# mlodel/gym-exploration-2d

Hardware: AMD Instinct MI355X
Metric: env-steps/sec (whole node), 4096 worlds x 10 agents (higher is better)
Workload: dtype f64; 1 GPU; 4096 worlds x 10 agents per GPU, RVO/ORCA on-device LP policy + OtherAgentsStates sensor, UnicycleDynamics, random-goal episodes with auto-reset (BASELINE configs[2]); worlds_per_gpu=4096, agents=10, launch_mode=cagym_rollout, parallelism=worlds sharded x1, no data-path collective

## Files before the change

### gym-exploration-2d_amd/csrc/cagym_api.hip

```cpp
#include <hip/hip_runtime.h>
#include <cmath>
#include <cstdio>
#include <cstdlib>
#include <algorithm>
#include <cstring>
#include <string>
#include <vector>

#include "../../include/cagym.h"
#include "cagym_gen1.h"
#include "cagym_sensors.h"
#include "cagym_kernels3.h"
#include "cagym_split3.h"
#include "cagym_launch3.h"
#ifdef CAGYM_MONOLITHIC
#include "cagym_k3_all.inc"
#endif
#include "cagym_ig.h"
#include "cagym_ga3c.h"
#include "cagym_ga3c16.h"
#include "cagym_gen.h"
#include "cagym_gen2.h"
#include "cagym_dmcts.h"
#include "cagym_ig_episode.h"
// ... 10 lines not shown
struct Env {
    cagym_config cfg;
    CagymDev D;
    std::vector<void*> allocs;
    std::string err;
    bool scenarios_set = false;
    double* sc_obst = nullptr;
    float4* sc_obst_prep = nullptr;
    double* sc_heading_buf = nullptr;
    IgDev G{};
    uint32_t* ig_any = nullptr;
    IgEpisode ig_ep{};
    int32_t* gen_failed = nullptr;
    int32_t* ga3c_ctr = nullptr;
    unsigned char* ga3c_packed = nullptr;
    const float* ga3c_packed_src = nullptr;
    int32_t* status_host = nullptr;
    bool ig_ready = false;
    int any_rvo = 1;
    int obst_rvo = 0;
    int generation = 3;
    int wpw10 = 5;
    size_t pre_lds_min = 0;
    bool begun = false;
    EpRec rec{};
    bool rec_ready = false;
    EpLog elog{};
    bool log_ready = false;
    void* elog_ring = nullptr;
    int n_ig = 0;
    bool streaming = false;
    StreamDev stream{};
    cagym_gen2_params stream_P{};
};
enum { N_IG_UNEQUAL = -1, N_IG_RANDOM = -2 };

int fail(Env* e, int code, const std::string& msg) {
    g_last_error = msg;
    if (e) e->err = msg;
    return code;
}

#define HIPCHK(e, call)                                                                              \
    do {                                                                                             \
        hipError_t _s = (call);                                                                      \
        if (_s != hipSuccess)                                                                        \
            return fail(e, CAGYM_E_HIP, std::string(#call) + ": " + hipGetErrorString(_s));          \
    } while (0)

struct DeviceGuard {
    int prev = -1;
    bool switched = false;
    hipError_t status = hipSuccess;
    explicit DeviceGuard(int dev) {
        status = hipGetDevice(&prev);
        if (status == hipSuccess && prev != dev) {
            status = hipSetDevice(dev);
            switched = status == hipSuccess;
        }
    }
    ~DeviceGuard() {
        if (switched) (void)hipSetDevice(prev);
    }
};
#define ENTRY_IF(e, env, state_ok, msg)                                \
    Env* e = reinterpret_cast<Env*>(env);                              \
    if (!e) return fail(nullptr, CAGYM_E_INVALID, "null env");         \
    if (!(state_ok)) return fail(e, CAGYM_E_STATE, msg)
#define ENTRY(e, env) ENTRY_IF(e, env, true, "")
#define ENTRY_POOL(e, env, name) ENTRY_IF(e, env, e->scenarios_set, name " before cagym_set_scenarios")
#define ENTRY_IG(e, env, name) ENTRY_IF(e, env, e->ig_ready, name " before cagym_ig_init")
#define ON_DEVICE(e)                                                                                       \
    DeviceGuard _guard((e)->cfg.device);                                                                   \
    if (_guard.status != hipSuccess) return fail(e, CAGYM_E_HIP, std::string("hipSetDevice: ") + hipGetErrorString(_guard.status)); \
    if (int _rc = device_status(e)) return _rc
#define ON_DEVICE_VOIDS_BEGUN(e) \
    ON_DEVICE(e);                \
    (e)->begun = false

int device_status(Env* e) {
    const int32_t code = e->status_host ? *reinterpret_cast<volatile int32_t*>(e->status_host) : 0;
    if (code == CAGYM_DEVERR_NONE) return CAGYM_OK;
    return fail(e, CAGYM_E_DEVICE, std::string("a kernel of an earlier launch gave up a bounded wait (") +
                                       (code == CAGYM_DEVERR_LP_WAIT ? "LP waves" : code == CAGYM_DEVERR_LASER_WAIT ? "LaserScan passes" : "unknown") +
                                       "): results since then are void, destroy the handle");
}

template <typename T>
int dalloc(Env* e, T** p, size_t n) {
    void* q = nullptr;
    size_t bytes = (n ? n : 1) * sizeof(T);
    hipError_t s = hipMalloc(&q, bytes);
    if (s != hipSuccess) return fail(e, CAGYM_E_NOMEM, std::string("hipMalloc: ") + hipGetErrorString(s));
    s = hipMemset(q, 0, bytes);
    if (s != hipSuccess) return fail(e, CAGYM_E_HIP, std::string("hipMemset: ") + hipGetErrorString(s));
    e->allocs.push_back(q);
    *p = reinterpret_cast<T*>(q);
    return CAGYM_OK;
}

CagymOut to_out(const Env* e, const cagym_outputs* o, bool scan_as_given = false) {
    CagymOut r{};
    if (o) {
        r.obs_oas = o->obs_oas;
        r.obs_ego = o->obs_ego;
        r.laserscan = (e->cfg.laserscan || scan_as_given) ? o->laserscan : nullptr;
        r.reward = o->reward;
        r.flags = o->flags;
        r.game_over = o->game_over;
    }
    return r;
}

#define WPW20 2
#define NT20 256
struct Spec2 {
    int nt, mt, wpw;
};
inline Spec2 spec2(int M, int wpw10) {
    if (M == 10) return {256, 10, wpw10};
    if (M == 4) return {256, 4, 0};
    if (M == 20) return {NT20, 20, WPW20};
    if (M <= 12) return {256, 0, 0};
    return {512, 0, 0};
}
inline Spec2 spec2(const Env* e) { return spec2(e->cfg.max_agents, e->wpw10); }
inline int wpw_spec(const Env* e) { return spec2(e).wpw; }
inline int n_wg2(const Env* e) {
    const int M = e->cfg.max_agents;
    const int wpw = wpw_spec(e) ? wpw_spec(e) : CAGYM_WAVE / M;
    return (e->cfg.n_worlds + wpw - 1) / wpw;
}
inline size_t lds3_bytes(const cagym_config& cfg, const Spec2 sp, bool obst, bool lines) {
    const int M = cfg.max_agents;
    return cagym_lds3_bytes(M, cagym_as(M, sp.wpw), sp.nt, (obst && lines) ? 2 * cfg.max_obstacles : 0, cagym_lpl3(sp.mt, obst), obst, sp.mt);
}
inline size_t lds3_bytes(const Env* e, bool obst, bool lines) { return lds3_bytes(e->cfg, spec2(e), obst, lines); }
inline bool has_map(const Env* e) { return e->cfg.max_obstacles > 0; }
inline size_t scan_bytes(const Env* e) { return (size_t)e->cfg.n_worlds * e->cfg.max_agents * 16 * sizeof(float); }
inline size_t lds3_bytes(const Env* e) { return lds3_bytes(e, has_map(e), e->obst_rvo != 0); }
inline size_t lds3_step_bytes(const Env* e) {
    if (!has_map(e)) return lds3_bytes(e);
    return cagym_lds3_ovl_bytes(e->cfg.max_agents, cagym_as(e->cfg.max_agents, wpw_spec(e)), spec2(e).nt, e->D.ko);
}
inline int lp_group_width(const Env* e) {
    const int mt = spec2(e).mt;
    return cagym_gw3(mt);
}

inline int n_waves(const Env* e) {
    int wpw = CAGYM_WAVE / e->cfg.max_agents;
    return (e->cfg.n_worlds + wpw - 1) / wpw;
}

struct K3Entry {
    int nt, mt, wp;
    void (*launch[2])(const K3Launch&);
    void (*setattr[2])(int);
};
#define K3_ROW(NT, MT, WP)                                                                     \
    {NT, MT, WP, {cagym_k3_launch_##NT##_##MT##_##WP##_0, cagym_k3_launch_##NT##_##MT##_##WP##_1}, \
     {cagym_k3_setattr_##NT##_##MT##_##WP##_0, cagym_k3_setattr_##NT##_##MT##_##WP##_1}},
const K3Entry k3_table[] = {CAGYM_K3_SPECS(K3_ROW)};
#undef K3_ROW
inline const K3Entry* k3_entry(const Env* e) {
    const Spec2 sp = spec2(e);
    for (const K3Entry& r : k3_table)
// ... 1444 lines not shown
```

### gym-exploration-2d_amd/csrc/cagym_kernels3.h

```cpp
#pragma once
#include "cagym_device.h"
#include "cagym_orca.h"

#include "cagym_spin.h"
#include "cagym_trace.h"

#ifndef CAGYM_GW10
#define CAGYM_GW10 8
#endif

__host__ __device__ inline size_t a16(size_t x) { return (x + 15) & ~(size_t)15; }

__device__ __forceinline__ void prio_chain3(bool lagging) {
#ifndef CAGYM_NO_LAG_PRIORITY
    if (lagging) __builtin_amdgcn_s_setprio(3);
    else __builtin_amdgcn_s_setprio(1);
#endif
}
__device__ __forceinline__ void prio_rows3() {
#ifndef CAGYM_NO_LAG_PRIORITY
    __builtin_amdgcn_s_setprio(0);
#endif
}
__host__ __device__ constexpr int cagym_gw3(int MT) { return MT > 0 && MT <= 5 ? 4 : (MT > 0 && MT <= 10 ? CAGYM_GW10 : 16); }
// ... 498 lines not shown
        if (!skip) gp = d - cr;
        klo = d - rl - rh;
        khi = d - rh - rl;
        const float rpx = (float)phx - (float)plx, rpy = (float)phy - (float)ply;
        dq = rpx * rpx + rpy * rpy;
    }
    W.hit[lo * MP + shi] = ht;
    W.hit[hi * MP + slo] = ht;
    if (GAP && gp < INFINITY) atomicMin(&W.gmin[lo], gap_key(gp));
    W.keys[lo * MP + shi] = klo;
    W.keys[hi * MP + slo] = khi;
    if (DSQ) {
        W.dsq[lo * MP + shi] = make_uint2((uint32_t)shi, __float_as_uint(dq));
        W.dsq[hi * MP + slo] = make_uint2((uint32_t)slo, __float_as_uint(dq));
    }
}

template <int MT>
__device__ __forceinline__ void pair_dsq3(const Lds3& W, int p, int M, int MP) {
    const UPair q = upair_of<MT>(p, M);
    const int n = W.wn[q.wl];
    const int lo = q.wl * M + (q.i < q.j ? q.i : q.j), hi = q.wl * M + (q.i < q.j ? q.j : q.i);
    const int slo = lo - q.wl * M, shi = hi - q.wl * M;
    float dq = INFINITY;
    if (shi < n) {
        const float rpx = (float)W.tpx[hi] - (float)W.tpx[lo], rpy = (float)W.tpy[hi] - (float)W.tpy[lo];
        dq = rpx * rpx + rpy * rpy;
    }
    W.dsq[lo * MP + shi] = make_uint2((uint32_t)shi, __float_as_uint(dq));
    W.dsq[hi * MP + slo] = make_uint2((uint32_t)slo, __float_as_uint(dq));
}

template <int MT>
__device__ __forceinline__ int neighbour_rank3(const Lds3& W, int a, int sl, float dq, int MP) {
    const uint4* row = reinterpret_cast<const uint4*>(W.dsq + a * MP);
    const unsigned long long me = ((unsigned long long)__float_as_uint(dq) << 32) | (unsigned)sl;
    int rank = 0;
    constexpr int MPT = MT > 0 ? ((MT + 1) & ~1) : 0;
    if (MT > 0) {
#pragma unroll
        for (int l2 = 0; l2 < MPT; l2 += 2) {
            const uint4 v = row[l2 >> 1];
            rank += ((((unsigned long long)v.y << 32) | v.x) < me) ? 1 : 0;
            rank += ((((unsigned long long)v.w << 32) | v.z) < me) ? 1 : 0;
        }
    } else {
        for (int l2 = 0; l2 < MP; l2 += 2) {
            const uint4 v = row[l2 >> 1];
            rank += ((((unsigned long long)v.y << 32) | v.x) < me) ? 1 : 0;
            rank += ((((unsigned long long)v.w << 32) | v.z) < me) ? 1 : 0;
        }
    }
    return rank;
}

template <int MT>
__device__ __forceinline__ void half_planes3(const CagymDev& D, const Lds3& W, int p, int M, int MP, int AS, int ko) {
    const UPair q = upair_of<MT>(p, M);
    const int n = W.wn[q.wl];
    const int a = q.wl * M + q.i, b = q.wl * M + q.j;
    const bool both = q.i < n && q.j < n;
    const bool on_a = both && W.trvo[a] != 0;
    const bool on_b = both && W.trvo[b] != 0;
    if (!(on_a || on_b)) return;
    const float vax = (float)W.tvx[a], vay = (float)W.tvy[a];
    const OrcaPair g = orca_pair((float)W.tpx[a], (float)W.tpy[a], vax, vay, (float)((1 + 15e-2) * W.tr[a]), (float)D.dt,
                                 W.tpx[b], W.tpy[b], W.tvx[b], W.tvy[b], W.tr[b]);
    PMARK("hp_pair_done");
    if (on_a) {
        const float c = W.tcoop[a];
        const float4 ln = make_float4(vax + c * g.ux, vay + c * g.uy, g.zx, g.zy);
        const float2 s0 = W.lpc[a];
        if (detf(ln.z, ln.w, ln.x - s0.x, ln.y - s0.y) > 0.0f) W.busy[a] = 1;
        const int rank = neighbour_rank3<MT>(W, a, q.j, g.d2, MP);
        if (rank < D.maxnb) W.sorted[(ko + rank) * AS + a] = ln;
    }
    if (on_b) {
        const float c = W.tcoop[b];
        const float4 ln = make_float4((float)W.tvx[b] - c * g.ux, (float)W.tvy[b] - c * g.uy, -g.zx, -g.zy);
        const float2 s0 = W.lpc[b];
        if (detf(ln.z, ln.w, ln.x - s0.x, ln.y - s0.y) > 0.0f) W.busy[b] = 1;
        const int rank = neighbour_rank3<MT>(W, b, q.i, g.d2, MP);
        if (rank < D.maxnb) W.sorted[(ko + rank) * AS + b] = ln;
    }
}

__device__ __forceinline__ void oas_row3(const Lds3& W, float* oas_out, int p, int npairs, int M, int MP, int K, int wpw,
                                         int worlds_valid, uint32_t inv_m) {
    PMARK("oas_begin");
    if (p >= npairs) return;
    const PairIdx q = pair_of(p, M, inv_m);
    if (q.j == q.sl || q.wl >= worlds_valid) return;
    const int n = W.wn[q.wl];
    float* my = oas_out + ((size_t)blockIdx.x * wpw * M + q.a) * K * 10;
    const double kj = W.keys[q.a * MP + q.j];
    if (!(kj > -INFINITY)) {
        const int row = q.sl < n ? q.j - 1 : (q.j < q.sl ? q.j : q.j - 1);
        float2* r2 = reinterpret_cast<float2*>(my + row * 10);
        const float2 z = make_float2(0.f, 0.f);
#pragma unroll
        for (int c = 0; c < 5; c++) r2[c] = z;
        return;
    }
    int before = 0;
    const double2* krow = reinterpret_cast<const double2*>(W.keys + q.a * MP);
    for (int l2 = 0; l2 < M; l2 += 2) {
        const double2 kk = krow[l2 >> 1];
        before += (kk.x > kj) || (kk.x == kj && l2 + 0 > q.j);
        before += (kk.y > kj) || (kk.y == kj && l2 + 1 > q.j);
    }
    const int row = before;
    PMARK("oas_ranked");
    const int b = q.a - q.sl + q.j;
    const double dx = W.tpx[b] - W.tpx[q.a], dy = W.tpy[b] - W.tpy[q.a];
    const double prx = W.tprx[q.a], pry = W.tpry[q.a], orx = -pry, ory = prx;
    const double ovx = W.tvx[b], ovy = W.tvy[b], orad = W.tr[b];
    float v[10];
    v[0] = (float)dx;
    v[1] = (float)dy;
    v[2] = (float)dot2(dx, dy, prx, pry);
    v[3] = (float)dot2(dx, dy, orx, ory);
    v[4] = (float)dot2(ovx, ovy, prx, pry);
    v[5] = (float)dot2(ovx, ovy, orx, ory);
    v[6] = (float)orad;
    v[7] = (float)(W.tr[q.a] + orad);
    v[8] = (float)kj;
    v[9] = ST_POLICY(W.tst[b]) == CAGYM_POL_STATIC ? 1.f : 2.f;
    PMARK("oas_store");
    float2* r2 = reinterpret_cast<float2*>(my + row * 10);
#pragma unroll
    for (int c = 0; c < 5; c++) r2[c] = make_float2(v[2 * c], v[2 * c + 1]);
}

__device__ __forceinline__ void ego_obs3(const CagymDev& D, const Lds3& W, float* ego_out, int a, int M, int wpw, uint32_t inv_m) {
    if (a >= wpw * M) return;
    const int wl = (int)__umulhi((uint32_t)a, inv_m);
    const int slot = a - wl * M;
    const int world = blockIdx.x * wpw + wl;
    if (world >= D.N) return;
    const int n = W.wn[wl];
    const bool active = slot < n;
    const int nobs = active ? n - 1 : 0;
    const size_t aidx = (size_t)world * M + slot;
    D.n_observed[aidx] = nobs;
    if (!ego_out) return;
    float4* e = reinterpret_cast<float4*>(ego_out + aidx * CAGYM_EGO_WIDTH);
    if (active) {
        const double px = W.tpx[a], py = W.tpy[a];
        e[0] = make_float4((float)W.tdg[a], (float)(W.tgx[a] - px), (float)(W.tgy[a] - py), (float)W.tr[a]);
        e[1] = make_float4((float)W.the[a], (float)W.th[a], (float)px, (float)py);
        e[2] = make_float4((float)W.tpref[a], (float)nobs, ST_POLICY(W.tst[a]) == CAGYM_POL_LEARNING ? 1.f : 0.f, 0.f);
    } else {
        const float4 z = make_float4(0.f, 0.f, 0.f, 0.f);
        e[0] = z; e[1] = z; e[2] = z;
    }
}

template <bool LEAN>
__device__ __forceinline__ bool sample_cell(double x, double y, int& gx, int& gy) {
    if (!LEAN) return world_to_cell(x, y, gx, gy);
    const double qy = y * 10.0, qx = x * 10.0;
    const bool safe = fabs(qy - rint(qy)) > 1e-7 && fabs(qx - rint(qx)) > 1e-7 && fabs(qy) < 1e6 && fabs(qx) < 1e6;
    if (!safe) return world_to_cell(x, y, gx, gy);
    gx = (int)floor((30 / 2.) / 0.1 - qy);
    gy = (int)floor((30 / 2.) / 0.1 + qx);
    return gx >= 0 && gy >= 0 && gx < CAGYM_MAPD && gy < CAGYM_MAPD;
// ... 118 lines not shown
            rng[i] = (uint8_t)((klo << 4) | khi);
        }
        cnt[c] = (uint8_t)__popcll(m);
    }
    WGTRACE_W1(30);
    if (!lds_wait_ge(&W.flag[8], npass)) *D.dev_status = CAGYM_DEVERR_LASER_WAIT;
    int n = 0;
    for (int q = 0; q < npass; q++) n += cnt[q];
    WGTRACE_W1_VALUE(32, n);
    for (;;) {
        int r = 0;
        if (lane == 0) r = __hip_atomic_fetch_add(&W.flag[10], 1, __ATOMIC_RELAXED, __HIP_MEMORY_SCOPE_WORKGROUP);
        r = __builtin_amdgcn_readlane(r, 0);
        if (r * CAGYM_WAVE >= n) break;
        int i = r * CAGYM_WAVE + lane;
        if (i < n) {
            int q = 0;
            for (; q < npass; q++) {
                const int cq = cnt[q];
                if (i < cq) break;
                i -= cq;
            }
            const int e = lst[q * CAGYM_WAVE + i], kk = rng[q * CAGYM_WAVE + i];
            const int a = e >> 4, b = e & 15;
            const int wl = (int)__umulhi((uint32_t)a, inv_m);
            const int slot = a - wl * M;
            const int world = blockIdx.x * wpw + wl;
            const uint32_t* map = D.map_bits + (size_t)W.wsc[wl] * CAGYM_MAPD * CAGYM_MAPW;
            laser_out[((size_t)world * M + slot) * 16 + b] = laserscan_beam_range<BATCH>(map, W.tpx[a], W.tpy[a], W.th[a], W.tr[a], b, kk >> 4, kk & 15);
        }
    }
    WGTRACE_W1(31);
}

template <bool OBST, int BATCH = 8>
__device__ __forceinline__ void observation_chunks3(const CagymDev& D, const Lds3& W, const CagymOut& o, int npairs, int M, int MP,
                                                    int K, int wpw, int worlds_valid, uint32_t inv_m, int ko = 0, int AS = 0) {
    const int lane = threadIdx.x & (CAGYM_WAVE - 1);
    const int nck = (npairs + CAGYM_WAVE - 1) / CAGYM_WAVE;
    for (;;) {
        int c = 0;
        if (lane == 0) c = __hip_atomic_fetch_add(&W.flag[1], 1, __ATOMIC_RELAXED, __HIP_MEMORY_SCOPE_WORKGROUP);
        c = __builtin_amdgcn_readlane(c, 0);
        if (c > nck) break;
        if (c < nck) {
            if (o.obs_oas) oas_row3(W, o.obs_oas, c * CAGYM_WAVE + lane, npairs, M, MP, K, wpw, worlds_valid, inv_m);
        } else {
            ego_obs3(D, W, o.obs_ego, lane, M, wpw, inv_m);
        }
    }
    if (OBST && o.laserscan) laser_scan3<BATCH>(D, W, o.laserscan, M, wpw, AS, inv_m, ko);
}

__device__ __forceinline__ CagymOut out_rows_slice3(const CagymOut& out, int t, size_t NM, int M) {
    CagymOut o;
    o.obs_oas = out.obs_oas ? out.obs_oas + (size_t)t * NM * (M - 1) * 10 : nullptr;
    o.obs_ego = out.obs_ego ? out.obs_ego + (size_t)t * NM * CAGYM_EGO_WIDTH : nullptr;
    o.laserscan = out.laserscan ? out.laserscan + (size_t)t * NM * 16 : nullptr;
    o.reward = nullptr; o.flags = nullptr; o.game_over = nullptr;
    return o;
}
__device__ __forceinline__ CagymOut out_slice3(const CagymOut& out, int t, size_t N, size_t NM, int M) {
    CagymOut o;
    o.obs_oas = out.obs_oas ? out.obs_oas + (size_t)t * NM * (M - 1) * 10 : nullptr;
    o.obs_ego = out.obs_ego ? out.obs_ego + (size_t)t * NM * CAGYM_EGO_WIDTH : nullptr;
    o.laserscan = out.laserscan ? out.laserscan + (size_t)t * NM * 16 : nullptr;
    o.reward = out.reward ? out.reward + (size_t)t * NM : nullptr;
    o.flags = out.flags ? out.flags + (size_t)t * NM : nullptr;
    o.game_over = out.game_over ? out.game_over + (size_t)t * N : nullptr;
    return o;
}

template <int NT, int MT, int WPWT, bool AUTO_RESET, bool OBST, bool ONE = false, bool POST = false>
__device__ inline void run_steps3(const CagymDev& D, unsigned char* smem, const float* ext, const CagymOut& out, int n_steps,
                                  bool any_rvo) {
    constexpr int NWAVES = NT / CAGYM_WAVE;
    constexpr int GW = cagym_gw3(MT), NG = NT / GW, NGW = CAGYM_WAVE / GW;
    constexpr bool TWO = cagym_two3(MT);
    constexpr int NL = TWO ? 2 * GW : GW + 1;
    const int M = MT ? MT : D.M, K = M - 1, MP = cagym_mp(M);
    const int AS = cagym_as(M, WPWT);
    const int ko = OBST ? D.ko : 0;
    constexpr int LPL = cagym_lpl3(MT, OBST);
    constexpr bool OVL = ONE && OBST && !POST;
    const Lds3 W = POST ? carve_lds3_post(smem, M, AS, ko / 2) : OVL ? carve_lds3_ovl(smem, M, AS, NT, ko) : carve_lds3(smem, M, AS, NT, ko, LPL, OBST, MT);
    const bool dsq_shared = !ONE && (OBST ? cagym_obst_alias(M, AS, NT, ko, LPL) : cagym_dsq_aliased(false, MT));
    LaneCtx C = make_ctx2(D, M, WPWT ? WPWT : CAGYM_WAVE / M);
    const uint32_t inv_m = (uint32_t)(0x100000000ull / (uint32_t)M) + 1u;
    const int nagents = C.wpw * M;
    const int npairs = C.wpw * M * M;
    const int nup = C.wpw * (M * (M - 1) / 2);
    const size_t NM = (size_t)D.N * M;
    float ep_ret = 0.f;
    int ep_len = 0;
    STAMP_BEGIN();
    {
        const int tid = threadIdx.x;
        const bool agent_lane = tid < nagents;
        if (!agent_lane) C.valid = C.active = false;
        if (agent_lane) {
            Agent A = {};
            if (C.valid) {
                load_agent(D, A, (size_t)C.world * M + C.slot);
                if (C.slot == 0) { ep_ret = D.ep_return[C.world]; ep_len = D.ep_len[C.world]; }
            }
            lds3_store_agent(W, A, tid);
            W.tmoved[tid] = 0;
            W.trvo[tid] = live_rvo(A.st, C.valid && C.active);
            W.nobl[tid] = 0;
            if (!OVL) W.gmin[tid] = CAGYM_GAP_INF;
            if (C.wl < C.wpw && C.slot == 0) {
                W.wn[C.wl] = C.valid ? C.n : 0;
                W.wsc[C.wl] = C.valid ? (int)(((long long)C.world + (long long)C.episode * D.N) % D.S) : 0;
            }
            if (!POST && !OVL) W.dsq[tid * MP + C.slot] = make_uint2((uint32_t)C.slot, 0x7f800000u);
            if (!OVL) {
                W.hit[tid * MP + C.slot] = 0;
                W.keys[tid * MP + C.slot] = -INFINITY;
            }
            for (int l = M; l < MP; l++) {
                if (!POST && !OVL) W.dsq[tid * MP + l] = make_uint2((uint32_t)l, 0x7f800000u);
                if (!OVL) {
                    W.hit[tid * MP + l] = 0;
                    W.keys[tid * MP + l] = -INFINITY;
                }
            }
        }
        if (tid < 16) W.flag[tid] = 0;
        __syncthreads();
        WGTRACE1(20);
        if (OBST && ko > 0) {
            stage_rects3(D, W, C.wpw, C.worlds_valid);
            __syncthreads();
        }
        WGTRACE1(21);
        if (agent_lane && any_rvo) ego_lp_inputs3<OBST>(D, W, tid, M, AS, ko, inv_m);
        else if (agent_lane) publish_pref_velocity3(W, tid);
        if (OBST && ko > 0 && any_rvo) {
            __syncthreads();
            obstacle_lines_phase3(D, W, M, AS, ko, nagents, inv_m);
        }
        WGTRACE1(22);
        if (any_rvo) {
            if (OVL && agent_lane) {
                W.dsq[tid * MP + C.slot] = make_uint2((uint32_t)C.slot, 0x7f800000u);
                for (int l = M; l < MP; l++) W.dsq[tid * MP + l] = make_uint2((uint32_t)l, 0x7f800000u);
            }
            for (int p = tid; p < nup; p += NT) {
                if (ONE) pair_dsq3<MT>(W, p, M, MP);
                else pair_distances3<MT, false>(D, W, p, M, MP);
            }
            __syncthreads();
            WGTRACE1(23);
            for (int p = tid; p < nup; p += NT) half_planes3<MT>(D, W, p, M, MP, AS, ko);
        }
        __syncthreads();
    }
    WGTRACE(1);
    bool lagging = false;
#pragma nounroll
    for (int t = 0; t < n_steps; t++) {
        int tid = threadIdx.x;
        asm volatile("" : "+v"(tid));
        const int wave = tid >> 6;
        const bool agent_lane = tid < nagents;
        int aidx32 = C.world * M + C.slot;
// ... 54 lines not shown
        }
        STAMP(1);
        WGTRACE1(24);
        PMARK("D_begin");
        Agent A;
        bool moved = false;
        const bool s1_lane = agent_lane && C.valid && C.active;
        if (wave == 0) {
            if (lp_waves > 0 && !lds_wait_ge(&W.flag[2], lp_waves)) *D.dev_status = CAGYM_DEVERR_LP_WAIT;
            STAMP(2);
            WAVETRACE(t, 3);
            PMARK("D_s1_begin");
            if (s1_lane) {
                A = lds3_load_agent(W, tid);
                float a0 = 0.f, a1 = 0.f;
                HeadingHint hint;
                hint.valid = false;
                if (!(A.st & CAGYM_FLAG_DONE)) {
                    double d0 = 0.0, d1 = 0.0;
                    switch (ST_POLICY(A.st)) {
                        case CAGYM_POL_STATIC: break;
                        case CAGYM_POL_NONCOOP: d0 = A.pref; d1 = -A.he; break;
                        case CAGYM_POL_EXTERNAL: case CAGYM_POL_IGMCTS: case CAGYM_POL_GA3C:
                            if (ext) { d0 = (double)ext[2 * aidx]; d1 = (double)ext[2 * aidx + 1]; }
                            break;
                        case CAGYM_POL_LEARNING:
                            if (ext) { d1 = 4.0 * (2. * (double)ext[2 * aidx + 1] - 1.); d0 = A.pref * (double)ext[2 * aidx]; }
                            else { d1 = -4.0; }
                            break;
                        case CAGYM_POL_CARRL: d0 = 1.0; d1 = carrl_heading(ext ? (int)ext[2 * aidx] : 0); break;
                        case CAGYM_POL_RVO: {
                            float2 v;
                            if (POST) v = D.lp_vel[aidx];
                            else v = W.lpc[tid];
                            orca_post(A, v.x, v.y, D.dt, D.inv_dt, d0, d1, &hint);
                            break;
                        }
                    }
                    a0 = (float)d0;
                    a1 = (float)d1;
                }
                asm volatile("" :: "v"(a0), "v"(a1));
                WAVETRACE(t, 15);
                if (TWO && !OBST && !POST) {
                    HeadingHint* hl = reinterpret_cast<HeadingHint*>(W.lp3) + tid;
                    *hl = hint;
                    asm volatile("" ::: "memory");
                    moved = take_action<false>(A, a0, a1, D.dt, hl);
                } else
                moved = take_action<false>(A, a0, a1, D.dt, &hint);
            }
            PMARK("D_s1_end");
            STAMP(3);
            WAVETRACE(t, 4);
        } else if (t > 0) {
            prio_rows3();
            PMARK("D_rows_begin");
            const CagymOut o_prev = out_rows_slice3(out, t - 1, NM, M);
            observation_chunks3<OBST, (ONE ? 8 : CAGYM_LASER_BATCH_ROLLOUT)>(D, W, o_prev, npairs, M, MP, K, C.wpw, C.worlds_valid, inv_m, ko, AS);
            prio_chain3(lagging);
            WAVETRACE(t, 4);
        }
        PMARK("D_end_barrierX");
        __syncthreads();
        WGTRACE1(25);
        WAVETRACE(t, 5);
        if (s1_lane) {
            lds3_store_s1(W, A, tid);
            W.tmoved[tid] = moved ? 1 : 0;
            W.trvo[tid] = live_rvo(A.st, true);
        } else if (agent_lane) {
            W.tmoved[tid] = 0;
        }
        if (OVL && agent_lane) {
            W.gmin[tid] = CAGYM_GAP_INF;
            W.hit[tid * MP + C.slot] = 0;
            W.keys[tid * MP + C.slot] = -INFINITY;
            for (int l = M; l < MP; l++) {
                W.hit[tid * MP + l] = 0;
                W.keys[tid * MP + l] = -INFINITY;
            }
        }
        if (tid == NT - 1) { W.flag[1] = 0; W.flag[2] = 0; W.flag[4] = W.flag[3]; W.flag[3] = 0; W.flag[7] = 0; W.flag[8] = 0; W.flag[9] = 0; W.flag[10] = 0; }
        __syncthreads();
        WGTRACE1(26);
        STAMP(4);
        WAVETRACE(t, 6);
        PMARK("A_begin");
        if (tid >= NT - CAGYM_WAVE) {
            const int a = tid - (NT - CAGYM_WAVE);
            if (a < nagents && any_rvo && t + 1 < n_steps) ego_lp_inputs3<OBST>(D, W, a, M, AS, ko, inv_m);
            WAVETRACE(t, 7);
        }
        if (OBST && D.map_bits && agent_lane) wall_prep3(D, W, tid, ko, inv_m, M);
        if (dsq_shared && agent_lane) {
            W.dsq[tid * MP + C.slot] = make_uint2((uint32_t)C.slot, 0x7f800000u);
            for (int l = M; l < MP; l++) W.dsq[tid * MP + l] = make_uint2((uint32_t)l, 0x7f800000u);
        }
        PMARK("A_pairs_begin");
        for (int p = tid; p < nup; p += NT) pair_distances3<MT, true, !ONE>(D, W, p, M, MP);
        PMARK("A_pairs_end");
        WAVETRACE(t, 8);
        const bool obst_lines = OBST && ko > 0 && any_rvo && t + 1 < n_steps;
        if (OBST && (D.map_bits || obst_lines)) __syncthreads();
        WGTRACE1(40);
        if (OBST && D.map_bits) wall_rows3<NWAVES>(D, W, nagents, inv_m);
        WGTRACE1(41);
        if (obst_lines) obstacle_lines_phase3(D, W, M, AS, ko, nagents, inv_m);
        __syncthreads();
        WGTRACE1(27);
        STAMP(5);
        WAVETRACE(t, 9);
        PMARK("B_begin");
        const bool more = t + 1 < n_steps;
        const int full_pairs = nup - nup % (NT - CAGYM_WAVE), tail_pairs = nup - full_pairs;
        if (wave == 0) {
            if (agent_lane) {
                float reward = 0.f;
                Agent S;
                S.st = W.tst[tid];
                const double dmin = gap_of_key(W.gmin[tid]);
                W.gmin[tid] = CAGYM_GAP_INF;
                if (C.valid && C.active) {
                    S.px = W.tpx[tid]; S.py = W.tpy[tid]; S.r = W.tr[tid];
                    bool coll_wall = false;
                    uint32_t hits = 0;
                    const uint32_t* hrow = reinterpret_cast<const uint32_t*>(W.hit + tid * MP);
                    for (int l4 = 0; l4 < MP; l4 += 4) hits |= hrow[l4 >> 2];
                    const bool coll_agent = hits != 0;
                    if (OBST && D.map_bits) coll_wall = W.lpk[tid] != 0;
                    double r = -0.01;
                    if (S.st & CAGYM_FLAG_AT_GOAL) {
                        if (!(S.st & CAGYM_FLAG_WAS_AT_GOAL)) r = 3.0;
                    } else {
                        if (!(S.st & CAGYM_FLAG_WAS_IN_COLLISION)) {
                            if (coll_agent) { r = -10.0; S.st |= CAGYM_FLAG_IN_COLLISION; }
                            else if (coll_wall) { r = -0.25; S.st |= CAGYM_FLAG_IN_COLLISION; }
                            else if (dmin <= 0.2) r += -0.1 - dmin / 2.;
                        } else if (S.st & CAGYM_FLAG_RAN_OUT_OF_TIME) {
                            r += -10.0;
                        }
                    }
                    r = clipd(r, -10.0, 3.0) / (3.0 - (-10.0));
                    reward = (float)r;
                    if (S.st & (CAGYM_FLAG_AT_GOAL | CAGYM_FLAG_RAN_OUT_OF_TIME | CAGYM_FLAG_IN_COLLISION)) S.st |= CAGYM_FLAG_DONE;
                }
                const bool live = C.valid && C.active;
                const bool done = !live || (S.st & CAGYM_FLAG_DONE);
                const uint64_t wm = world_mask64(C);
                const uint64_t b_done = __ballot(done);
                const uint64_t b_learn = __ballot(done || ST_POLICY(S.st) != CAGYM_POL_LEARNING);
                bool go;
                if (D.go_mode == CAGYM_GO_ALL) go = (b_done & wm) == wm;
                else if (D.go_mode == CAGYM_GO_LEARNING) go = (b_learn & wm) == wm;
                else go = C.n > 0 ? ((b_done >> C.base) & 1ull) : true;
                if (C.valid) {
                    const size_t ot = (size_t)t * NM;
                    if (out.reward) out.reward[ot + aidx] = reward;
                    if (out.flags) out.flags[ot + aidx] = (uint8_t)(S.st & 0xffu);
                    if (C.slot == 0) {
                        if (out.game_over) out.game_over[(size_t)t * (size_t)D.N + C.world] = go ? 1 : 0;
                        ep_ret += reward;
                        ep_len += 1;
                    }
                }
                bool any_reset = false;
                if (AUTO_RESET) {
                    const bool rs = C.valid && go;
                    any_reset = __ballot(rs) != 0ull;
                    if (any_reset) {
                        float r0 = rs ? ep_ret : 0.f;
                        int l0 = rs ? ep_len : 0;
                        LaneCtx Cr = C;
                        Cr.valid = rs;
                        asm volatile("" : "+v"(Cr.world));
                        fold_episode_stats(D, Cr, S, r0, l0);
                        if (rs) {
                            ep_ret = 0.f;
                            ep_len = 0;
                            C.episode += 1;
                            int sidx = (int)(((long long)C.world + (long long)C.episode * D.N) % D.S);
                            C.n = D.sc_nagents[sidx];
                            C.active = C.slot < C.n;
                            init_agent(D, S, sidx, C.slot, C.active);
                            lds3_store_agent(W, S, tid);
                            if (C.slot == 0) {
                                int wlq = C.wl;
                                asm volatile("" : "+v"(wlq));
                                W.wn[wlq] = C.n;
                                W.wsc[wlq] = sidx;
                            }
                        }
                    }
                }
                W.tst[tid] = S.st;
                if (tid == 0) W.flag[0] = any_reset ? 1 : 0;
                if (W.tmoved[tid] && !(AUTO_RESET && C.valid && go)) {
                    Agent E;
                    E.px = W.tpx[tid]; E.py = W.tpy[tid]; E.gx = W.tgx[tid]; E.gy = W.tgy[tid]; E.h = W.th[tid];
                    double prx, pry;
                    update_ego_frame(E, prx, pry);
                    W.tdg[tid] = E.dg; W.the[tid] = E.he; W.tprx[tid] = prx; W.tpry[tid] = pry;
                }
            }
            PMARK("B_s2_end");
            if (any_rvo && more && tail_pairs <= CAGYM_WAVE && tid < tail_pairs) half_planes3<MT>(D, W, full_pairs + tid, M, MP, AS, ko);
        } else if (any_rvo && more) {
            const int lim = tail_pairs <= CAGYM_WAVE ? full_pairs : nup;
            PMARK("B_hp_begin");
            for (int p = tid - CAGYM_WAVE; p < lim; p += NT - CAGYM_WAVE) half_planes3<MT>(D, W, p, M, MP, AS, ko);
        }
        if (OBST && ONE && out.laserscan) {
            laser_scan3<8>(D, W, out.laserscan, M, C.wpw, AS, inv_m, ko);
        }
        PMARK("B_end");
        WAVETRACE(t, 10);
        __syncthreads();
        WGTRACE1(28);
        STAMP(6);
        WAVETRACE(t, 11);
        PMARK("R_begin");
        const int f_reset = W.flag[0], f_lag = W.flag[4];
        lagging = __builtin_amdgcn_readfirstlane(f_lag) != 0;
        if (AUTO_RESET && f_reset) {
            if (OBST && tid == 0) { W.flag[7] = 0; W.flag[8] = 0; W.flag[9] = 0; W.flag[10] = 0; }
            if (OBST && ko > 0) {
                stage_rects3(D, W, C.wpw, C.worlds_valid);
                __syncthreads();
            }
            if (tid >= NT - CAGYM_WAVE) {
                const int a = tid - (NT - CAGYM_WAVE);
                if (a < nagents) {
                    const int wl = (int)__umulhi((uint32_t)a, inv_m);
                    W.trvo[a] = live_rvo(W.tst[a], (a - wl * M) < W.wn[wl]);
                    if (any_rvo && more) ego_lp_inputs3<OBST>(D, W, a, M, AS, ko, inv_m);
                }
            }
            for (int p = tid; p < nup; p += NT) pair_distances3<MT, false, !ONE>(D, W, p, M, MP);
            if (OBST && ko > 0 && any_rvo && more) {
                __syncthreads();
                obstacle_lines_phase3(D, W, M, AS, ko, nagents, inv_m);
            }
            __syncthreads();
            if (any_rvo && more)
                for (int p = tid; p < nup; p += NT) half_planes3<MT>(D, W, p, M, MP, AS, ko);
            __syncthreads();
        }
        PMARK("step_end");
        STAMP(7);
        WAVETRACE(t, 12);
        WGTRACE(2 + t);
    }
    {
        CagymOut o_last = out_slice3(out, n_steps - 1, (size_t)D.N, NM, M);
        if (OBST && ONE && !W.flag[0]) o_last.laserscan = nullptr;
        observation_chunks3<OBST, (ONE ? 8 : CAGYM_LASER_BATCH_ROLLOUT)>(D, W, o_last, npairs, M, MP, K, C.wpw, C.worlds_valid, inv_m, ko, AS);
        if (C.valid) {
            const Agent A = lds3_load_agent(W, threadIdx.x);
            store_agent(D, A, (size_t)C.world * M + C.slot, true);
            if (C.slot == 0) {
                D.ep_return[C.world] = ep_ret;
                D.ep_len[C.world] = ep_len;
                D.episode[C.world] = C.episode;
                D.n_agents[C.world] = C.n;
            }
        }
    }
}

#ifndef CAGYM_MINW_WIDE
#define CAGYM_MINW_WIDE 4
#endif
__host__ __device__ constexpr int cagym_min_waves3(int NT, int MT) { return NT > 256 ? 2 : ((MT > 0 && MT <= 10) ? 4 : CAGYM_MINW_WIDE); }

template <int NT, int MT, int WPWT, bool AUTO_RESET, bool OBST>
__global__ void __launch_bounds__(NT, OBST ? 2 : cagym_min_waves3(NT, MT)) k_rollout3(CagymDev D, int n_steps, CagymOut out, int any_rvo) {
    extern __shared__ __attribute__((aligned(16))) unsigned char smem[];
    WGTRACE(0);
    WGTRACE_VALUE(39, 0);
    if (OBST) { [[clang::always_inline]] run_steps3<NT, MT, WPWT, AUTO_RESET, OBST>(D, smem, nullptr, out, n_steps, any_rvo != 0); }
    else run_steps3<NT, MT, WPWT, AUTO_RESET, OBST>(D, smem, nullptr, out, n_steps, any_rvo != 0);
    WGTRACE(38);
    WGTRACE_XCC();
}

template <int NT, int MT, int WPWT, bool AUTO_RESET, bool OBST>
__global__ void __launch_bounds__(NT, OBST ? (NT > 256 ? 2 : 4) : cagym_min_waves3(NT, MT)) k_step3(CagymDev D, const float* ext, CagymOut out, int any_rvo) {
    extern __shared__ __attribute__((aligned(16))) unsigned char smem[];
    WGTRACE(0);
    WGTRACE_VALUE(39, 0);
// ... 5 lines not shown
```

### gym-exploration-2d_amd/csrc/cagym_spin.h

```cpp
#pragma once

#ifndef CAGYM_SPIN_HD
#ifdef __HIPCC__
#define CAGYM_SPIN_HD __host__ __device__ __forceinline__
#else
#define CAGYM_SPIN_HD inline
#endif
#endif

#define CAGYM_SPIN_LIMIT (1u << 20)

enum { CAGYM_DEVERR_NONE = 0, CAGYM_DEVERR_LP_WAIT = 1, CAGYM_DEVERR_LASER_WAIT = 2 };

template <typename Load, typename Pause>
CAGYM_SPIN_HD bool cagym_bounded_wait(Load load, int target, unsigned limit, Pause pause) {
    for (unsigned i = 0; i < limit; i++) {
        if (load() >= target) return true;
        pause();
    }
    return load() >= target;
}

#ifdef __HIPCC__
__device__ __forceinline__ bool lds_wait_ge(int* ctr, int target) {
    return cagym_bounded_wait([&]() { return __hip_atomic_load(ctr, __ATOMIC_ACQUIRE, __HIP_MEMORY_SCOPE_WORKGROUP); }, target,
                              CAGYM_SPIN_LIMIT, []() { __builtin_amdgcn_s_sleep(1); });
}
#endif
```

Measured before the change: 511.0 million env-steps/s.

## Fuse ego-frame and pair phases with LDS flag sync instead of barriers

For fixed small agent counts without obstacles, wave 0 computes ego-frame and LP inputs while the other waves compute pairwise distances, hit flags and ORCA half-planes in one pass. LDS atomic counters with bounded spin waits replace the block barriers between phases, and half-plane construction moves from phase B into phase A. This aims to remove barrier stalls and a separate half-plane loop, at the cost of spin-wait overhead and a new device error code if a wait times out.

Measured after the change: 518.3 million env-steps/s, median of 6. 1.4% higher.

```diff
diff --git a/gym-exploration-2d_amd/csrc/cagym_api.hip b/gym-exploration-2d_amd/csrc/cagym_api.hip
--- a/gym-exploration-2d_amd/csrc/cagym_api.hip
+++ b/gym-exploration-2d_amd/csrc/cagym_api.hip
@@ -116,7 +116,7 @@
     const int32_t code = e->status_host ? *reinterpret_cast<volatile int32_t*>(e->status_host) : 0;
     if (code == CAGYM_DEVERR_NONE) return CAGYM_OK;
     return fail(e, CAGYM_E_DEVICE, std::string("a kernel of an earlier launch gave up a bounded wait (") +
-                                       (code == CAGYM_DEVERR_LP_WAIT ? "LP waves" : code == CAGYM_DEVERR_LASER_WAIT ? "LaserScan passes" : "unknown") +
+                                       (code == CAGYM_DEVERR_LP_WAIT ? "LP waves" : code == CAGYM_DEVERR_LASER_WAIT ? "LaserScan passes" : code == CAGYM_DEVERR_PAIR_WAIT ? "pair phase" : "unknown") +
                                        "): results since then are void, destroy the handle");
 }
 
diff --git a/gym-exploration-2d_amd/csrc/cagym_kernels3.h b/gym-exploration-2d_amd/csrc/cagym_kernels3.h
--- a/gym-exploration-2d_amd/csrc/cagym_kernels3.h
+++ b/gym-exploration-2d_amd/csrc/cagym_kernels3.h
@@ -604,6 +604,111 @@
         if (detf(ln.z, ln.w, ln.x - s0.x, ln.y - s0.y) > 0.0f) W.busy[b] = 1;
         const int rank = neighbour_rank3<MT>(W, b, q.i, g.d2, MP);
         if (rank < D.maxnb) W.sorted[(ko + rank) * AS + b] = ln;
+    }
+}
+
+template <bool LP>
+__device__ __forceinline__ void ego_phase3(const Lds3& W, int a) {
+    const double px = W.tpx[a], py = W.tpy[a], tgx = W.tgx[a], tgy = W.tgy[a], h = W.th[a];
+    const bool mv = W.tmoved[a] != 0;
+    float ox = 0.f, oy = 0.f, radius = 0.f;
+    if (LP) {
+        const double gx = tgx - px, gy = tgy - py;
+        const double pref = W.tpref[a];
+        const double sc = pref / norm2(gx, gy);
+        ox = (float)(sc * gx); oy = (float)(sc * gy); radius = (float)pref;
+    }
+    Agent E;
+    E.px = px; E.py = py; E.gx = tgx; E.gy = tgy; E.h = h;
+    double prx, pry;
+    update_ego_frame(E, prx, pry);
+    if (LP) {
+        W.lpv[a] = make_float2(ox, oy);
+        W.lpr[a] = radius;
+        float cx = ox, cy = oy;
+        if (ox * ox + oy * oy > radius * radius) {
+            const float inv = 1.0f / sqrtf(ox * ox + oy * oy);
+            cx = ox * inv * radius;
+            cy = oy * inv * radius;
+        }
+        W.lpc[a] = make_float2(cx, cy);
+        W.busy[a] = 0;
+    }
+    if (mv) { W.tdg[a] = E.dg; W.the[a] = E.he; W.tprx[a] = prx; W.tpry[a] = pry; }
+}
+
+template <int MT, bool PLANES>
+__device__ __forceinline__ void pair_phase3(const CagymDev& D, const Lds3& W, int p, bool has, int M, int MP, int AS, int pair_waves, int t) {
+    UPair q = {0, 0, 0};
+    int a = 0, b = 0;
+    bool both = false;
+    bool on_a = false, on_b = false;
+    OrcaPair g = {0.f, 0.f, 0.f, 0.f, 0.f};
+    float vax = 0.f, vay = 0.f, vbx = 0.f, vby = 0.f, ca = 0.f, cb = 0.f;
+    if (has) {
+        q = upair_of<MT>(p, M);
+        const int n = W.wn[q.wl];
+        a = q.wl * M + q.i;
+        b = q.wl * M + q.j;
+        both = q.i < n && q.j < n;
+        const int lo = q.i < q.j ? a : b, hi = q.i < q.j ? b : a;
+        double kab = -INFINITY, kba = -INFINITY, gp = INFINITY;
+        float dq = INFINITY;
+        uint8_t ht = 0;
+        if (both) {
+            const double pax = W.tpx[a], pay = W.tpy[a], pbx = W.tpx[b], pby = W.tpy[b];
+            const double ra = W.tr[a], rb = W.tr[b];
+            const uint32_t st_hi = W.tst[hi];
+            double dvax = 0., dvay = 0., dvbx = 0., dvby = 0.;
+            if (PLANES) {
+                dvax = W.tvx[a]; dvay = W.tvy[a]; dvbx = W.tvx[b]; dvby = W.tvy[b];
+                on_a = W.trvo[a] != 0;
+                on_b = W.trvo[b] != 0;
+                ca = W.tcoop[a];
+                cb = W.tcoop[b];
+            }
+            const double dx = pbx - pax, dy = pby - pay;
+            const double d = norm2(dx, dy);
+            const bool skip = ST_POLICY(st_hi) == CAGYM_POL_STATIC && !D.collide_static;
+            const double cr = ra + rb;
+            ht = (!skip && d <= cr) ? 1 : 0;
+            if (!skip) gp = d - cr;
+            kab = d - ra - rb;
+            kba = d - rb - ra;
+            const float rpx = (float)pbx - (float)pax, rpy = (float)pby - (float)pay;
+            dq = rpx * rpx + rpy * rpy;
+            if (PLANES) {
+                vax = (float)dvax; vay = (float)dvay; vbx = (float)dvbx; vby = (float)dvby;
+                g = orca_pair((float)pax, (float)pay, vax, vay, (float)((1 + 15e-2) * ra), (float)D.dt, pbx, pby, dvbx, dvby, rb);
+            }
+        }
+        W.hit[a * MP + q.j] = ht;
+        W.hit[b * MP + q.i] = ht;
+        if (gp < INFINITY) atomicMin(&W.gmin[lo], gap_key(gp));
+        W.keys[a * MP + q.j] = kab;
+        W.keys[b * MP + q.i] = kba;
+        W.dsq[a * MP + q.j] = make_uint2((uint32_t)q.j, __float_as_uint(dq));
+        W.dsq[b * MP + q.i] = make_uint2((uint32_t)q.i, __float_as_uint(dq));
+    }
+    if ((threadIdx.x & (CAGYM_WAVE - 1)) == 0) __hip_atomic_fetch_add(&W.flag[11], 1, __ATOMIC_RELEASE, __HIP_MEMORY_SCOPE_WORKGROUP);
+    WAVETRACE(t, 8);
+    if (!PLANES) return;
+    PMARK("hp_pair_done");
+    if (!lds_wait_ge(&W.flag[11], pair_waves) || !lds_wait_ge(&W.flag[12], 1)) *D.dev_status = CAGYM_DEVERR_PAIR_WAIT;
+    WAVETRACE(t, 9);
+    if (on_a) {
+        const float4 ln = make_float4(vax + ca * g.ux, vay + ca * g.uy, g.zx, g.zy);
+        const float2 s0 = W.lpc[a];
+        if (detf(ln.z, ln.w, ln.x - s0.x, ln.y - s0.y) > 0.0f) W.busy[a] = 1;
+        const int rank = neighbour_rank3<MT>(W, a, q.j, g.d2, MP);
+        if (rank < D.maxnb) W.sorted[rank * AS + a] = ln;
+    }
+    if (on_b) {
+        const float4 ln = make_float4(vbx - cb * g.ux, vby - cb * g.uy, -g.zx, -g.zy);
+        const float2 s0 = W.lpc[b];
+        if (detf(ln.z, ln.w, ln.x - s0.x, ln.y - s0.y) > 0.0f) W.busy[b] = 1;
+        const int rank = neighbour_rank3<MT>(W, b, q.i, g.d2, MP);
+        if (rank < D.maxnb) W.sorted[rank * AS + b] = ln;
     }
 }
 
@@ -888,6 +993,8 @@
     const int AS = cagym_as(M, WPWT);
     const int ko = OBST ? D.ko : 0;
     constexpr int LPL = cagym_lpl3(MT, OBST);
+    constexpr int WPWC = WPWT ? WPWT : (MT > 0 ? CAGYM_WAVE / MT : 0);
+    constexpr bool FUSED = !OBST && !ONE && !POST && MT > 0 && NT > CAGYM_WAVE && WPWC * (MT * (MT - 1) / 2) <= NT - CAGYM_WAVE;
     constexpr bool OVL = ONE && OBST && !POST;
     const Lds3 W = POST ? carve_lds3_post(smem, M, AS, ko / 2) : OVL ? carve_lds3_ovl(smem, M, AS, NT, ko) : carve_lds3(smem, M, AS, NT, ko, LPL, OBST, MT);
     const bool dsq_shared = !ONE && (OBST ? cagym_obst_alias(M, AS, NT, ko, LPL) : cagym_dsq_aliased(false, MT));
@@ -1108,11 +1215,32 @@
             }
         }
         if (tid == NT - 1) { W.flag[1] = 0; W.flag[2] = 0; W.flag[4] = W.flag[3]; W.flag[3] = 0; W.flag[7] = 0; W.flag[8] = 0; W.flag[9] = 0; W.flag[10] = 0; }
+        if (FUSED && tid == NT - 1) { W.flag[11] = 0; W.flag[12] = 0; }
         __syncthreads();
         WGTRACE1(26);
         STAMP(4);
         WAVETRACE(t, 6);
         PMARK("A_begin");
+        if constexpr (FUSED) {
+            const bool more = t + 1 < n_steps;
+            if (wave == 0) {
+                if (agent_lane) {
+                    if (any_rvo && more) ego_phase3<true>(W, tid);
+                    else ego_phase3<false>(W, tid);
+                }
+                if (dsq_shared && agent_lane) {
+                    W.dsq[tid * MP + C.slot] = make_uint2((uint32_t)C.slot, 0x7f800000u);
+                    for (int l = M; l < MP; l++) W.dsq[tid * MP + l] = make_uint2((uint32_t)l, 0x7f800000u);
+                }
+                if (tid == 0) __hip_atomic_fetch_add(&W.flag[12], 1, __ATOMIC_RELEASE, __HIP_MEMORY_SCOPE_WORKGROUP);
+                WAVETRACE(t, 7);
+                if (!lds_wait_ge(&W.flag[11], NWAVES - 1)) *D.dev_status = CAGYM_DEVERR_PAIR_WAIT;
+                WAVETRACE(t, 9);
+            } else {
+                if (any_rvo && more) pair_phase3<MT, true>(D, W, tid - CAGYM_WAVE, tid - CAGYM_WAVE < nup, M, MP, AS, NWAVES - 1, t);
+                else pair_phase3<MT, false>(D, W, tid - CAGYM_WAVE, tid - CAGYM_WAVE < nup, M, MP, AS, NWAVES - 1, t);
+            }
+        } else {
         if (tid >= NT - CAGYM_WAVE) {
             const int a = tid - (NT - CAGYM_WAVE);
             if (a < nagents && any_rvo && t + 1 < n_steps) ego_lp_inputs3<OBST>(D, W, a, M, AS, ko, inv_m);
@@ -1134,9 +1262,10 @@
         WGTRACE1(41);
         if (obst_lines) obstacle_lines_phase3(D, W, M, AS, ko, nagents, inv_m);
         __syncthreads();
+        WAVETRACE(t, 9);
+        }
         WGTRACE1(27);
         STAMP(5);
-        WAVETRACE(t, 9);
         PMARK("B_begin");
         const bool more = t + 1 < n_steps;
         const int full_pairs = nup - nup % (NT - CAGYM_WAVE), tail_pairs = nup - full_pairs;
@@ -1221,7 +1350,7 @@
                 }
                 W.tst[tid] = S.st;
                 if (tid == 0) W.flag[0] = any_reset ? 1 : 0;
-                if (W.tmoved[tid] && !(AUTO_RESET && C.valid && go)) {
+                if (!FUSED && W.tmoved[tid] && !(AUTO_RESET && C.valid && go)) {
                     Agent E;
                     E.px = W.tpx[tid]; E.py = W.tpy[tid]; E.gx = W.tgx[tid]; E.gy = W.tgy[tid]; E.h = W.th[tid];
                     double prx, pry;
@@ -1230,8 +1359,8 @@
                 }
             }
             PMARK("B_s2_end");
-            if (any_rvo && more && tail_pairs <= CAGYM_WAVE && tid < tail_pairs) half_planes3<MT>(D, W, full_pairs + tid, M, MP, AS, ko);
-        } else if (any_rvo && more) {
+            if (!FUSED && any_rvo && more && tail_pairs <= CAGYM_WAVE && tid < tail_pairs) half_planes3<MT>(D, W, full_pairs + tid, M, MP, AS, ko);
+        } else if (!FUSED && any_rvo && more) {
             const int lim = tail_pairs <= CAGYM_WAVE ? full_pairs : nup;
             PMARK("B_hp_begin");
             for (int p = tid - CAGYM_WAVE; p < lim; p += NT - CAGYM_WAVE) half_planes3<MT>(D, W, p, M, MP, AS, ko);
diff --git a/gym-exploration-2d_amd/csrc/cagym_spin.h b/gym-exploration-2d_amd/csrc/cagym_spin.h
--- a/gym-exploration-2d_amd/csrc/cagym_spin.h
+++ b/gym-exploration-2d_amd/csrc/cagym_spin.h
@@ -10,7 +10,7 @@
 
 #define CAGYM_SPIN_LIMIT (1u << 20)
 
-enum { CAGYM_DEVERR_NONE = 0, CAGYM_DEVERR_LP_WAIT = 1, CAGYM_DEVERR_LASER_WAIT = 2 };
+enum { CAGYM_DEVERR_NONE = 0, CAGYM_DEVERR_LP_WAIT = 1, CAGYM_DEVERR_LASER_WAIT = 2, CAGYM_DEVERR_PAIR_WAIT = 3 };
 
 template <typename Load, typename Pause>
 CAGYM_SPIN_HD bool cagym_bounded_wait(Load load, int target, unsigned limit, Pause pause) {
```
